# biotite-dev/springcraft

Measured on AMD Instinct MI355X. Metric: ANM modes/sec (Hessian build + full eigensolve), N=2000 C-alpha, higher is better.
Workload: dtype f64; 1 GPU; C3: N=2000 C-alpha ANM, HinsenForceField (no cutoff), full 6000x6000 eigensolve, all modes + vectors; parallelism=independent structures sharded over GPUs, no data-path collective

## Files before the change

### include/springcraft_hip_debug.h

```cpp
#ifndef SPRINGCRAFT_HIP_DEBUG_H
#define SPRINGCRAFT_HIP_DEBUG_H

#include "springcraft_hip.h"

#ifdef __cplusplus
extern "C" {
#endif

int sc_dbg_gemm_bench(sc_ctx* ctx, int m, int n, int k, int mode, int tile, int split_k, int iters, int beta_one,
                      double* ms_out, double* max_err_out);

int sc_dbg_gemm_host(sc_ctx* ctx, const double* a, const double* b, double* c, int m, int n, int k, int mode, int tile,
                     int split_k, double alpha, double beta, int lower_grid);

typedef struct sc_dbg_gemm_record {
  long long a, b, c;
  long long a_kidx, b_kidx, c_jidx;
  long long sa_i, sa_k, sb_k, sb_j, ldc, split_stride;
  double alpha, beta;
  int m, n, k;
  int lower_only, row_off, col_off;
  int a_tri;
  int reserved;
} sc_dbg_gemm_record;

int sc_dbg_gemm_records_host(sc_ctx* ctx, double* arena, long long arena_len, const int* idx, long long idx_len,
                             const sc_dbg_gemm_record* recs, int count, int max_m, int max_n, int split_k, int gather,
                             int tri, int layout, int lower_grid, int tile);

int sc_dbg_gemm3_host(sc_ctx* ctx, const double* a, const double* b, double* c, int count, int m, int n, int k, int layout,
                      int lower, double beta);

int sc_dbg_symm3_host(sc_ctx* ctx, const double* a, const double* v, double* x, int count, int m, int split);
int sc_dbg_symm3_stamps(unsigned long long* out4);
int sc_dbg_symm3_bench(sc_ctx* ctx, int count, int m, int split, int iters, double* ms_out);

int sc_dbg_gemm3_bench(sc_ctx* ctx, int count, int m, int n, int k, int layout, int lower, int kernel, int order, int iters,
                       double* ms_out);

int sc_dbg_gemm_stamps(unsigned long long* out4, int reset);

int sc_dbg_gemm_trace(unsigned long long* out, int max_records, int* count, int reset);

int sc_dbg_reduce_host(sc_ctx* ctx, const double* a, int n, int batch, int which, double* d_out, double* e_out,
                       double* scale_out, double* band_out, double* q_out, int* two_stage_out);

int sc_dbg_stedc_host(sc_ctx* ctx, const double* d, const double* e, int n, int batch, double* w_out, double* z_out);
int sc_dbg_stedc_leaf_max(int n);

int sc_dbg_partial_tridiag_host(sc_ctx* ctx, const double* d, const double* e, const double* f, const int* own, int n,
                                int batch, int window, int il, int m, double vl, double vu, int vectors, double* w_out,
                                double* z_out, int* win_out, long long* count_out);

int sc_dbg_bt2_stamps(unsigned long long* out);

int sc_dbg_bt2_clock(unsigned long long* out2);

int sc_dbg_bt2_trace(unsigned long long* out);

int sc_dbg_bulge_stamps(unsigned long long* out6);
int sc_dbg_pair_stamps(unsigned long long* out48);
int sc_dbg_chase_stamps(unsigned long long* out16);

int sc_dbg_set_chase(sc_ctx* ctx, int mode, int give_up_after);

int sc_dbg_set_panel_coop(sc_ctx* ctx, int min_rows);
int sc_dbg_set_panel_coop_fail(sc_ctx* ctx, int panel);

int sc_dbg_set_resident(sc_ctx* ctx, int mode, int hook, int workgroups);
int sc_dbg_resident_stamps(unsigned long long* out8);

#ifdef __cplusplus
}
#endif
#endif
```

### springcraft_amd/csrc/gemm_debug.hip

```cpp
#include <algorithm>
#include <cmath>
#include <cstdlib>
#include <vector>

#include "gemm_f64.h"
#include "springcraft_hip_debug.h"

namespace {
struct FirstError {
  sc_ctx* ctx;
  int rc = SC_OK;
  void operator()(hipError_t e) { if (e != hipSuccess && rc == SC_OK) rc = sc_set_error(ctx, SC_ERR_HIP, "%s", hipGetErrorString(e)); }
};

struct Shape {
  sc_ctx* ctx;
  int count;
  size_t ea, eb, ec;
  FirstError fail{ctx};
  char* base = nullptr;
  double *a = nullptr, *b = nullptr, *c = nullptr;
  GemmDesc* d = nullptr;
  ~Shape() { (void)hipFree(base); }
  int alloc() {
// ... 167 lines not shown
  if (R.ldc < R.m) return "ldc < m";
  if (R.k > 0) {
    if ((wide)R.a + (wide)(R.m - 1) * R.sa_i + (wide)ka * R.sa_k >= (wide)arena_len) return "A reaches outside the arena";
    if ((wide)R.b + (wide)kb * R.sb_k + (wide)(R.n - 1) * R.sb_j >= (wide)arena_len) return "B reaches outside the arena";
  }
  if ((wide)R.c + (wide)(L.split_k - 1) * R.split_stride + (wide)jc * R.ldc + (R.m - 1) >= (wide)arena_len)
    return "C reaches outside the arena";
  return nullptr;
}
}

extern "C" int sc_dbg_gemm_records_host(sc_ctx* ctx, double* arena, long long arena_len, const int* idx, long long idx_len,
                                        const sc_dbg_gemm_record* recs, int count, int max_m, int max_n, int split_k,
                                        int gather, int tri, int layout, int lower_grid, int tile) {
  if (!ctx) return SC_ERR_INVALID_ARG;
  if (!arena || arena_len <= 0 || arena_len > (1ll << 34) || idx_len < 0 || idx_len > (1ll << 34) || (idx_len > 0 && !idx) ||
      !recs || count < 0 || count > (1 << 24) || max_m <= 0 || max_n <= 0 || split_k < 1 || split_k > 65535)
    return sc_set_error(ctx, SC_ERR_INVALID_ARG, "GEMM records: bad launch argument");
  if (tile < 10 || tile > 13) return sc_set_error(ctx, SC_ERR_INVALID_ARG, "tile id %d (10 .. 13)", tile);
  if (layout < 0 || layout > 2 || (gather && (tri || layout != kGemmAmBk)) || (tri && layout == kGemmAmBn))
    return sc_set_error(ctx, SC_ERR_INVALID_ARG, "GEMM records: no kernel for layout %d, gather %d, tri %d", layout, gather, tri);
  if (lower_grid && (layout != kGemmAmBn || tri || gather || split_k > 1 || max_m != max_n))
    return sc_set_error(ctx, SC_ERR_INVALID_ARG, "GEMM records: lower_grid is for square launches of layout kGemmAmBn without split-K");
  const GemmLaunch L{.count = count, .max_m = max_m, .max_n = max_n, .layout = layout, .split_k = split_k, .gather = gather != 0,
                     .tri = tri != 0, .lower_grid = lower_grid != 0, .dbg = {.force_tile = tile - 10}};
  for (int r = 0; r < count; ++r) {
    const char* what = gemm_record_problem(recs[r], arena_len, idx, idx_len, L);
    if (what) return sc_set_error(ctx, SC_ERR_INVALID_ARG, "GEMM record %d: %s", r, what);
  }
  SC_HIP(ctx, hipSetDevice(ctx->device));
  auto up = [](size_t b) { return (b + 255) / 256 * 256; };
  const size_t b_arena = up((size_t)(arena_len + 2 * kRecGuard) * 8), b_desc = up((size_t)std::max(count, 1) * sizeof(GemmDesc));
  const size_t b_idx = up((size_t)std::max<long long>(idx_len, 1) * 4);
  char* base = nullptr;
  SC_HIP(ctx, hipMalloc((void**)&base, b_arena + b_desc + b_idx));
  double *d_front = (double*)base, *d_arena = d_front + kRecGuard, *d_back = d_arena + arena_len;
  GemmDesc* d_desc = (GemmDesc*)(base + b_arena);
  int* d_idx = (int*)(base + b_arena + b_desc);
  FirstError fail{ctx};
  std::vector<unsigned long long> guard((size_t)kRecGuard, kRecGuardBits), got((size_t)kRecGuard);
  fail(hipMemcpy(d_front, guard.data(), (size_t)kRecGuard * 8, hipMemcpyHostToDevice));
  fail(hipMemcpy(d_back, guard.data(), (size_t)kRecGuard * 8, hipMemcpyHostToDevice));
  fail(hipMemcpy(d_arena, arena, (size_t)arena_len * 8, hipMemcpyHostToDevice));
  if (idx_len > 0) fail(hipMemcpy(d_idx, idx, (size_t)idx_len * 4, hipMemcpyHostToDevice));
  std::vector<GemmDesc> h_desc((size_t)count);
  for (int r = 0; r < count; ++r) {
    const sc_dbg_gemm_record& R = recs[r];
    GemmDesc& D = h_desc[(size_t)r];
    D = GemmDesc{};
    D.a = d_arena + R.a; D.b = d_arena + R.b; D.c = d_arena + R.c;
    D.m = R.m; D.n = R.n; D.k = R.k;
    D.sa_i = R.sa_i; D.sa_k = R.sa_k; D.sb_k = R.sb_k; D.sb_j = R.sb_j; D.ldc = R.ldc;
    D.alpha = R.alpha; D.beta = R.beta;
    D.a_kidx = R.a_kidx >= 0 ? d_idx + R.a_kidx : nullptr;
    D.b_kidx = R.b_kidx >= 0 ? d_idx + R.b_kidx : nullptr;
    D.c_jidx = R.c_jidx >= 0 ? d_idx + R.c_jidx : nullptr;
    D.lower_only = R.lower_only; D.row_off = R.row_off; D.col_off = R.col_off;
    D.split_stride = R.split_stride; D.a_tri = R.a_tri;
  }
  if (count > 0) fail(hipMemcpy(d_desc, h_desc.data(), (size_t)count * sizeof(GemmDesc), hipMemcpyHostToDevice));
  if (fail.rc == SC_OK) {
    fail.rc = launch_gemm_f64(ctx, d_desc, L);
    fail(hipStreamSynchronize(ctx->stream));
  }
  if (fail.rc == SC_OK) fail(hipMemcpy(arena, d_arena, (size_t)arena_len * 8, hipMemcpyDeviceToHost));
  for (double* g : {d_front, d_back}) {
    if (fail.rc != SC_OK) break;
    fail(hipMemcpy(got.data(), g, (size_t)kRecGuard * 8, hipMemcpyDeviceToHost));
    if (fail.rc == SC_OK && got != guard) fail.rc = sc_set_error(ctx, SC_ERR_HIP, "GEMM records: the launch wrote outside the arena");
  }
  (void)hipFree(base);
  return fail.rc;
}

extern "C" int sc_dbg_gemm3_host(sc_ctx* ctx, const double* a, const double* b, double* c, int count, int m, int n, int k,
                                 int layout, int lower, double beta) {
  if (!ctx || !a || !b || !c || count < 1 || m < 1 || n < 1 || k < 1) return SC_ERR_INVALID_ARG;
  Shape S{ctx, count, (size_t)m * k, (size_t)k * n, (size_t)m * n};
  SC_TRY(S.alloc());
  S.fail(hipMemcpy(S.a, a, S.ea * count * 8, hipMemcpyHostToDevice));
  S.fail(hipMemcpy(S.b, b, S.eb * count * 8, hipMemcpyHostToDevice));
  S.fail(hipMemcpy(S.c, c, S.ec * count * 8, hipMemcpyHostToDevice));
  S.upload(gemm3_record(m, n, k, layout, lower, beta, m, n, m));
  if (S.fail.rc == SC_OK) {
    const int took = launch_gemm3_uniform(ctx, S.d, {.count = count, .m = m, .n = n, .k = k, .layout = layout, .lower = lower, .alpha = 1.0,
                                                     .beta = beta, .aligned16 = true, .dbg = {.any_size = true}});
    if (took != SC_OK) S.fail.rc = sc_set_error(ctx, SC_ERR_INVALID_ARG, "k_gemm3 does not take m %d n %d k %d layout %d", m, n, k, layout);
    S.fail(hipStreamSynchronize(ctx->stream));
  }
  if (S.fail.rc == SC_OK) S.fail(hipMemcpy(c, S.c, S.ec * count * 8, hipMemcpyDeviceToHost));
  return S.fail.rc;
}

extern "C" int sc_dbg_gemm3_bench(sc_ctx* ctx, int count, int m, int n, int k, int layout, int lower, int kernel, int order,
                                  int iters, double* ms_out) {
  if (!ctx || count < 1 || iters < 1) return SC_ERR_INVALID_ARG;
  static const int ld_a = [] { const char* e = getenv("SC_DBG_LDA"); return e ? atoi(e) : 0; }();
  static const int ld_c = [] { const char* e = getenv("SC_DBG_LDC"); return e ? atoi(e) : 0; }();
  static const int ld_b = [] { const char* e = getenv("SC_DBG_LDB"); return e ? atoi(e) : 0; }();
  const int lda = std::max(m, ld_a), ldc = std::max(m, ld_c), ldbn = std::max(n, ld_b);
  Shape S{ctx, count, (size_t)lda * k, layout == kGemmAmBn ? (size_t)ldbn * k : (size_t)k * n, (size_t)ldc * n};
  SC_TRY(S.alloc());
  S.fill_random();
  S.fail(hipMemset(S.c, 0, S.ec * count * 8));
  S.upload(gemm3_record(m, n, k, layout, lower, 1.0, lda, ldbn, ldc));
  if (S.fail.rc != SC_OK) return S.fail.rc;
  return S.time(2, iters, ms_out, [&]() -> int {
    if (kernel != 3)
      return launch_gemm_f64(ctx, S.d, {.count = count, .max_m = m, .max_n = n, .layout = layout, .lower_grid = lower != 0 && layout == kGemmAmBn});
    const int took = launch_gemm3_uniform(ctx, S.d, {.count = count, .m = m, .n = n, .k = k, .layout = layout, .lower = lower, .alpha = 1.0,
                                                     .beta = 1.0, .aligned16 = true, .dbg = {.any_size = true, .order = order}});
    return took == SC_OK ? SC_OK : SC_ERR_INVALID_ARG;
  });
}

extern "C" int sc_dbg_symm3_host(sc_ctx* ctx, const double* a, const double* v, double* x, int count, int m, int split) {
  if (!ctx || !a || !v || !x || count < 1 || m < 1 || split < 1) return SC_ERR_INVALID_ARG;
  const size_t ev = (size_t)m * 64;
  Shape S{ctx, count, (size_t)m * m, ev, ev * split};
  SC_TRY(S.alloc());
  S.fail(hipMemcpy(S.a, a, S.ea * count * 8, hipMemcpyHostToDevice));
  S.fail(hipMemcpy(S.b, v, ev * count * 8, hipMemcpyHostToDevice));
  S.fail(hipMemset(S.c, 0xff, S.ec * count * 8));
  S.upload(symm3_record(m));
  if (S.fail.rc == SC_OK) {
    const int took = launch_symm3(ctx, S.d, count, m, split, true, true);
    if (took != SC_OK) S.fail.rc = sc_set_error(ctx, SC_ERR_INVALID_ARG, "k_symm3 does not take m %d split %d", m, split);
    S.fail(hipStreamSynchronize(ctx->stream));
  }
  if (S.fail.rc == SC_OK) {
    std::vector<double> hx(S.ec * count);
    S.fail(hipMemcpy(hx.data(), S.c, hx.size() * 8, hipMemcpyDeviceToHost));
    for (int z = 0; z < count; ++z)
      for (size_t e = 0; e < ev; ++e) {
        double s = 0.0;
        for (int q = 0; q < split; ++q) s += hx[(size_t)z * S.ec + (size_t)q * ev + e];
        x[(size_t)z * ev + e] = s;
      }
  }
  return S.fail.rc;
}

extern "C" int sc_dbg_symm3_bench(sc_ctx* ctx, int count, int m, int split, int iters, double* ms_out) {
  if (!ctx || count < 1 || iters < 1 || m < 256) return SC_ERR_INVALID_ARG;
  Shape S{ctx, count, (size_t)m * m, (size_t)m * 64, (size_t)m * 64 * split};
  SC_TRY(S.alloc());
  S.fill_random();
  S.upload(symm3_record(m));
  if (S.fail.rc != SC_OK) return S.fail.rc;
  return S.time(2, iters, ms_out, [&] {
    return launch_symm3(ctx, S.d, count, m, split, true, true) == SC_OK ? SC_OK : SC_ERR_INVALID_ARG;
  });
}
```

### springcraft_amd/csrc/gemm_f64.h

```cpp
#pragma once

#include <cstdint>

#include "common.h"
#include "gemm_policy.h"

struct GemmDesc {
  const double* a;
  const double* b;
  double* c;
  int m, n, k;
  long long sa_i, sa_k;
  long long sb_k, sb_j;
  long long ldc;
  double alpha, beta;
  const int* a_kidx;
  const int* b_kidx;
  const int* c_jidx;
  int lower_only;
  int row_off, col_off;
  long long split_stride;
  int a_tri;
};

using sc_host::GemmLaunch, sc_host::Gemm3Launch, sc_host::GemmOverrides;
int launch_gemm_f64(sc_ctx* ctx, const GemmDesc* d_desc, const GemmLaunch& L);
int gemm_f64_tile(const sc_ctx* ctx, int count, int max_m, int max_n, int layout);
inline sc_host::GemmDevice gemm_device(const sc_ctx* ctx) { return {ctx->num_cus, ctx->gemm3_attr, ctx->gemm3_side_by_side}; }

int launch_gemm3_uniform(sc_ctx* ctx, const GemmDesc* d_desc, const Gemm3Launch& L);
bool gemm3_would_take(sc_ctx* ctx, const Gemm3Launch& L);

int launch_symm3(sc_ctx* ctx, const GemmDesc* d_desc, int count, int m, int split, bool aligned16, bool any_size);
bool symm3_would_take(sc_ctx* ctx, int count, int m, int split, bool aligned16);
```

### springcraft_amd/csrc/sy2sb.hip

```cpp
#include <algorithm>
#include <vector>

#include "twostage_internal.h"

namespace {

constexpr int kEarly = (kIb + 2) / 2;

__global__ __launch_bounds__(256) void k_panel_qr(double* __restrict__ a_all, long long stride_a,
                                                  double* __restrict__ tri_all, TriLayout TL,
                                                  double* __restrict__ sb_all, SbLayout SL, int j0, int j, int nr,
                                                  int c_end) {
  constexpr int LD = kQrRows + 1;
  extern __shared__ __attribute__((aligned(16))) double sm[];
  const int c_lo = j > 0 ? j - 1 : 0;
  const int ncl = c_end - c_lo;
  double* P = sm;
  double* wv = sm + ncl * LD;
  double* vv = wv + kB;
  double* red = vv + kQrRows;
  __shared__ double s_scale, s_beta, s_tau;

  const int n = TL.n;
  const int r0 = j0 + kB, m = n - r0;
// ... 1056 lines not shown
      GemmDesc P{};
      P.a = sb + SL.xv + (size_t)2 * kB * n + r0; P.sa_i = n; P.sa_k = 1;
      P.b = sb + SL.xv + r0; P.sb_k = 1; P.sb_j = n;
      P.c = sb + SL.small; P.ldc = kB;
      P.m = kB; P.n = 3 * kB; P.k = m; P.alpha = 1.0; P.beta = 0.0;
      P.split_stride = (long long)kB * 3 * kB;
      g[2] = P;
      GemmDesc W{};
      W.a = sb + SL.xv + r0; W.sa_i = 1; W.sa_k = n;
      W.b = sb + SL.cmat; W.sb_k = 1; W.sb_j = 3 * kB;
      W.c = sb + SL.vw + (size_t)vw_w * n + r0; W.ldc = n;
      W.m = m; W.n = kB; W.k = 3 * kB; W.alpha = 1.0; W.beta = 0.0;
      g[3] = W;
      W.c = sb + SL.wv + (size_t)wv_w * n + r0;
      W.alpha = -1.0;
      g[4] = W;
      GemmDesc R{};
      R.a = sb + SL.vw + r0; R.sa_i = 1; R.sa_k = n;
      R.b = sb + SL.wv + r0; R.sb_k = n; R.sb_j = 1;
      R.c = a22; R.ldc = n;
      R.m = m; R.n = m; R.k = rl == 2 ? 4 * kB : 2 * kB; R.alpha = 1.0; R.beta = 1.0;
      R.lower_only = sc_host::symm3_for(E, n) ? 2 : 1;
      g[5] = R;
      GemmDesc D = R;
      D.n = kB; D.k = 2 * kB;
      g[6] = D;
      GemmDesc Q{};
      Q.a = sb + SL.wv + r0; Q.sa_i = n; Q.sa_k = 1;
      Q.b = sb + SL.xv + (size_t)2 * kB * n + r0; Q.sb_k = 1; Q.sb_j = n;
      Q.c = sb + SL.small2; Q.ldc = 2 * kB;
      Q.m = 2 * kB; Q.n = kB; Q.k = m; Q.alpha = 1.0; Q.beta = 0.0;
      Q.split_stride = (long long)2 * kB * kB;
      g[7] = Q;
      GemmDesc Cr{};
      Cr.a = sb + SL.vw + r0; Cr.sa_i = 1; Cr.sa_k = n;
      Cr.b = sb + SL.p2; Cr.sb_k = 1; Cr.sb_j = 2 * kB;
      Cr.c = sb + SL.xv + r0; Cr.ldc = n;
      Cr.m = m; Cr.n = kB; Cr.k = 2 * kB; Cr.alpha = 1.0; Cr.beta = 1.0;
      g[8] = Cr;
    }
  }
  std::vector<GemmDesc> hs(h.size());
  for (int p = 0; p < npanels; ++p)
    for (int b = 0; b < batch; ++b) {
      const GemmDesc* g = &h[((size_t)p * batch + b) * kDescKinds];
      GemmDesc* o = &hs[(size_t)p * kDescKinds * batch];
      for (int kd = 0; kd < kDescKinds; ++kd) o[(size_t)kd * batch + b] = g[kd];
    }
  return hs;
}

struct PanelRun {
  sc_ctx* ctx;
  hipStream_t st;
  double* d_a; long long stride_a; int n, batch;
  double* d_tri_ws; const TriLayout& TL;
  double* d_sb_ws; const SbLayout& SL;
  const GemmDesc* d_descs;
  const std::vector<int>& role;
  sc_host::CoopPlan coop;
  v4i* coop_recs;
  int* coop_ctl;
  bool use_symm3;
  int symm3_nb_min;
  SbTimers& t;
};

static int run_panel(const PanelRun& R, int p, int lo, int hi, hipStream_t ps, bool timed) {
  using sc_host::PanelQr;
  const sc_host::TwoStageEnv& E = sc_host::two_stage_env();
  sc_ctx* ctx = R.ctx;
  const TriLayout& TL = R.TL;
  const SbLayout& SL = R.SL;
  const int n = R.n, batch = R.batch;
  const long long stride_a = R.stride_a;
  struct StreamScope {
    sc_ctx* c; hipStream_t old;
    StreamScope(sc_ctx* c_, hipStream_t s) : c(c_), old(c_->stream) { c->stream = s; }
    ~StreamScope() { c->stream = old; }
  } scope(ctx, ps);
  const int nb = hi - lo;
  const int rl = R.role[(size_t)p];
  double* a_h = R.d_a + (size_t)lo * stride_a;
  double* tri_h = R.d_tri_ws + (size_t)lo * TL.slab;
  double* sb_h = R.d_sb_ws + (size_t)lo * SL.slab;
  const int j0 = p * kB, r0 = j0 + kB, m = n - r0;
  const int nr = std::min(kB, m - 1);
  const int nchunks = (m + kQrRows - 1) / kQrRows;
  const dim3 qgrid((unsigned)nchunks, (unsigned)nb);
  SbLayout SQ = SL;
  if (rl == 2) { SQ.vw += (long long)2 * kB * n; SQ.wv += (long long)2 * kB * n; }
  if (timed) R.t.qr.start();
  const sc_host::PanelQrForm F = sc_host::panel_qr_form(E, R.coop, R.coop_recs != nullptr, m, nb, ps == R.st);
  switch (F.kind) {
    case PanelQr::Coop: {
      const int coop_g = F.coop_g;
      if (p == ctx->coop_fail_panel) SC_HIP(ctx, hipMemsetAsync(R.coop_ctl + 8 * lo, 1, sizeof(int) * 8 * nb, ps));
      hipLaunchKernelGGL(k_panel_coop, dim3((unsigned)coop_g, (unsigned)nb), dim3(kCoopRows), kCoopLdsBytes, ps, a_h, stride_a,
                         tri_h, TL, sb_h, SQ, j0, coop_g, R.coop_recs + (size_t)lo * coop_recs_per_matrix(coop_g),
                         R.coop_ctl + 8 * lo, (p + 1) * 128);
      hipLaunchKernelGGL(k_panel_serial, dim3((unsigned)nb), dim3(1024), 0, ps, a_h, stride_a, tri_h, TL, sb_h, SQ, j0,
                         (const int*)(R.coop_ctl + 8 * lo), ctx->d_status);
      ++ctx->cnt_coop_launches;
      break;
    }
    case PanelQr::Wg1024: {
      const size_t lds_wg = sizeof(double) * (size_t)(2 * kWgWaves * 8 + 16 + 8 + 8 * kB + kWgWaves * kB * 8);
      const dim3 g1((unsigned)nb), b1((unsigned)kWgThreads);
      ++ctx->cnt_panel_form[std::max(1, std::min(F.ru, 4)) - 1];
      if (F.ru == 1) hipLaunchKernelGGL((k_panel_wg<1, 8>), g1, b1, lds_wg, ps, a_h, stride_a, tri_h, TL, sb_h, SQ, j0);
      else if (F.ru == 2) hipLaunchKernelGGL((k_panel_wg<2, 8>), g1, b1, lds_wg, ps, a_h, stride_a, tri_h, TL, sb_h, SQ, j0);
      else if (F.ru == 3) hipLaunchKernelGGL((k_panel_wg<3, 4>), g1, b1, lds_wg, ps, a_h, stride_a, tri_h, TL, sb_h, SQ, j0);
      else hipLaunchKernelGGL((k_panel_wg<4, 2>), g1, b1, lds_wg, ps, a_h, stride_a, tri_h, TL, sb_h, SQ, j0);
      break;
    }
    case PanelQr::Wg512: {
      constexpr int kW = 512 / 64;
      const size_t lds_wg = sizeof(double) * (size_t)(2 * kW * 8 + 16 + 8 + 8 * kB + kW * kB * 8);
      const dim3 g1((unsigned)nb), b1(512u);
      ++ctx->cnt_panel_form[F.ru == 10 ? 4 : 5];
      if (F.ru == 10) hipLaunchKernelGGL((k_panel_wg<10, 1, 512>), g1, b1, lds_wg, ps, a_h, stride_a, tri_h, TL, sb_h, SQ, j0);
      else hipLaunchKernelGGL((k_panel_wg<12, 1, 512>), g1, b1, lds_wg, ps, a_h, stride_a, tri_h, TL, sb_h, SQ, j0);
      break;
    }
    case PanelQr::Blocked: {
      const size_t lds_qr_blk = sizeof(double) * ((size_t)(kIb + 1) * (kQrRows + 1) + kB + kQrRows + 4 * kB);
      const size_t lds_blk_a = sizeof(double) * ((size_t)kB * (kQrRows + 1) + kQrRows + 8 * kB);
      const size_t lds_blk_b = sizeof(double) * ((size_t)kB * (kQrRows + 1) + kIb * kB + 4 * kB);
      ++ctx->cnt_panel_form[6];
      hipLaunchKernelGGL(k_panel_qr, qgrid, dim3(256), lds_qr_blk, ps, a_h, stride_a, tri_h, TL, sb_h, SQ, j0, 0, nr, kIb);
      for (int c0 = 0; c0 < kB; c0 += kIb) {
        for (int j = c0 + 1; j < c0 + kIb; ++j)
          hipLaunchKernelGGL(k_panel_qr, qgrid, dim3(256), lds_qr_blk, ps, a_h, stride_a, tri_h, TL, sb_h, SQ, j0, j, nr,
                             c0 + kIb);
        const size_t cut = sizeof(double) * (size_t)c0 * (kQrRows + 1);
        hipLaunchKernelGGL(k_pqr_blk_a, qgrid, dim3(256), lds_blk_a - cut, ps, a_h, stride_a, tri_h, TL, sb_h, SQ, j0, c0);
        if (c0 + kIb < kB)
          hipLaunchKernelGGL(k_pqr_blk_b, qgrid, dim3(256), lds_blk_b - cut, ps, a_h, stride_a, tri_h, TL, sb_h, SQ, j0, c0);
      }
      break;
    }
    case PanelQr::Unblocked: {
      const size_t lds_qr = sizeof(double) * ((size_t)kB * (kQrRows + 1) + kB + kQrRows + 4 * kB);
      ++ctx->cnt_panel_form[7];
      for (int j = 0; j <= nr; ++j)
        hipLaunchKernelGGL(k_panel_qr, qgrid, dim3(256), lds_qr, ps, a_h, stride_a, tri_h, TL, sb_h, SQ, j0, j, nr, kB);
      break;
    }
  }
  if (timed) R.t.qr.stop();
  if (rl != 0) ++ctx->cnt_panel_role[rl - 1];
  const GemmDesc* g = R.d_descs + (size_t)p * kDescKinds * batch;
  if (timed) R.t.symm.start();
  if (R.use_symm3 && symm3_would_take(ctx, R.symm3_nb_min, m, SL.symm_split, true) &&
      launch_symm3(ctx, g + lo, nb, m, SL.symm_split, true, true) == SC_OK) {
    if (SL.symm_split > 1)
      hipLaunchKernelGGL(k_sum_xslices, dim3((unsigned)((m + 255) / 256), kB, (unsigned)nb), dim3(256), 0, ps, sb_h, SL, r0);
  } else {
    ++ctx->cnt_symm_tri;
    SC_TRY(launch_gemm_f64(ctx, g + lo, {.count = nb, .max_m = m, .max_n = kB, .layout = kGemmAmBk, .split_k = SL.symm_split, .tri = true}));
    SC_TRY(launch_gemm_f64(ctx, g + batch + lo, {.count = nb, .max_m = m, .max_n = kB, .layout = kGemmAkBk, .split_k = SL.symm_split, .tri = true}));
    if (SL.symm_split > 1)
      hipLaunchKernelGGL(k_sum_xslices, dim3((unsigned)((m + 255) / 256), 2 * kB, (unsigned)nb), dim3(256), 0, ps, sb_h, SL, r0);
  }
  if (rl == 2) {
    SC_TRY(launch_gemm_f64(ctx, g + 7 * batch + lo, {.count = nb, .max_m = 2 * kB, .max_n = kB, .layout = kGemmAkBk, .split_k = kSmallSplit}));
    hipLaunchKernelGGL(k_sum_p2, dim3((unsigned)(2 * kB * kB / 256), (unsigned)nb), dim3(256), 0, ps, sb_h, SL);
    SC_TRY(launch_gemm_f64(ctx, g + 8 * batch + lo, {.count = nb, .max_m = m, .max_n = kB, .layout = kGemmAmBk}));
  }
  if (timed) R.t.symm.stop();
  SC_TRY(launch_gemm_f64(ctx, g + 2 * batch + lo, {.count = nb, .max_m = kB, .max_n = 3 * kB, .layout = kGemmAkBk, .split_k = kSmallSplit}));
  const size_t lds_small = sizeof(double) * 4 * kB * (kB + 1);
  hipLaunchKernelGGL(k_sb_small, dim3((unsigned)nb), dim3(1024), lds_small, ps, tri_h, TL, sb_h, SL, j0);
  if (nb == batch) {
    SC_TRY(launch_gemm_f64(ctx, g + 3 * batch, {.count = 2 * batch, .max_m = m, .max_n = kB, .layout = kGemmAmBk}));
  } else {
    SC_TRY(launch_gemm_f64(ctx, g + 3 * batch + lo, {.count = nb, .max_m = m, .max_n = kB, .layout = kGemmAmBk}));
    SC_TRY(launch_gemm_f64(ctx, g + 4 * batch + lo, {.count = nb, .max_m = m, .max_n = kB, .layout = kGemmAmBk}));
  }
  if (timed) R.t.syr2k.start();
  if (rl == 1)
    SC_TRY(launch_gemm_f64(ctx, g + 6 * batch + lo, {.count = nb, .max_m = m, .max_n = kB, .layout = kGemmAmBn}));
  else
    if (launch_gemm3_uniform(ctx, g + 5 * batch + lo,
                             {.count = nb, .m = m, .n = m, .k = rl == 2 ? 4 * kB : 2 * kB, .layout = kGemmAmBn, .lower = R.use_symm3 ? 2 : 1,
                              .alpha = 1.0, .beta = 1.0, .aligned16 = (n & 1) == 0 && (r0 & 1) == 0}) != SC_OK) {
      ++ctx->cnt_gemm3_declined;
      SC_TRY(launch_gemm_f64(ctx, g + 5 * batch + lo, {.count = nb, .max_m = m, .max_n = m, .layout = kGemmAmBn, .lower_grid = true}));
    }
  if (timed) R.t.syr2k.stop();
  return SC_OK;
}

int sb_stage1(sc_ctx* ctx, double* d_a, long long stride_a, int n, int batch, double* d_tri_ws, const TriLayout& TL,
              double* d_sb_ws, const SbLayout& SL, const GemmDesc* d_descs, const std::vector<int>& role, bool prof,
              SbTimers& timers) {
  const sc_host::TwoStageEnv& E = sc_host::two_stage_env();
  hipStream_t st = ctx->stream;
  const int npanels = (int)role.size();

  for (int b = 0; b < batch; ++b)
    SC_HIP(ctx, hipMemsetAsync(d_tri_ws + (size_t)b * TL.slab + TL.tau, 0, sizeof(double) * n, st));

  const int s1_parts = sc_host::stage1_parts(E, batch, prof);
  ctx->last_stage1_parts = s1_parts;
  ctx->last_symm_slices = SL.symm_split;
  const sc_host::CoopPlan coop = sc_host::coop_plan(E, n, batch, ctx->num_cus, prof, ctx->coop_min_rows, ctx->coop_ok);
  v4i* coop_recs = nullptr;
  int* coop_ctl = nullptr;
  if (coop.ask) {
    if (ctx->coop_attr < 0)
      ctx->coop_attr = hipFuncSetAttribute(reinterpret_cast<const void*>(&k_panel_coop),
                                           hipFuncAttributeMaxDynamicSharedMemorySize, (int)kCoopLdsBytes) == hipSuccess;
    if (ctx->coop_attr == 1 && coop.nb_max >= 1) {
      const size_t rec_bytes = (size_t)batch * coop_recs_per_matrix(coop.gmax) * sizeof(v4i);
      const size_t ctl_bytes = align_up((size_t)batch * 8 * sizeof(int), 256);
      SC_TRY(sc_reserve_dc_aux(ctx, ctl_bytes + rec_bytes));
      coop_ctl = reinterpret_cast<int*>(ctx->dc_aux);
      coop_recs = reinterpret_cast<v4i*>(reinterpret_cast<char*>(ctx->dc_aux) + ctl_bytes);
      SC_HIP(ctx, hipMemsetAsync(ctx->dc_aux, 0, ctl_bytes + rec_bytes, st));
    }
  }
  const bool use_symm3 = sc_host::symm3_for(E, n);
  if (use_symm3)
    for (int b = 0; b < batch; ++b)
      SC_HIP(ctx, hipMemsetAsync(d_sb_ws + (size_t)b * SL.slab + SL.xv + (size_t)kB * n, 0, sizeof(double) * (size_t)kB * n, st));
  const PanelRun R{ctx, st, d_a, stride_a, n, batch, d_tri_ws, TL, d_sb_ws, SL, d_descs, role, coop, coop_recs, coop_ctl,
                   use_symm3, std::max(1, batch / s1_parts), timers};
  if (s1_parts > 1) {
    struct SideBySide {
      sc_ctx* c;
      explicit SideBySide(sc_ctx* c_) : c(c_) { c->gemm3_side_by_side = true; }
      ~SideBySide() { c->gemm3_side_by_side = false; }
    } side_by_side(ctx);
    SC_TRY(sc_aux_stream(ctx));
    SC_TRY(sc_side_streams(ctx, s1_parts - 1));
    SC_HIP(ctx, hipEventRecord(ctx->aux_fork, st));
    for (int q = 1; q < s1_parts; ++q) SC_HIP(ctx, hipStreamWaitEvent(ctx->side_streams[q - 1], ctx->aux_fork, 0));
    int rc_parts = SC_OK;
    for (int p = 0; p < npanels && rc_parts == SC_OK; ++p)
      for (int q = 0; q < s1_parts && rc_parts == SC_OK; ++q) {
        const int lo = (int)((long long)batch * q / s1_parts), hi = (int)((long long)batch * (q + 1) / s1_parts);
        rc_parts = run_panel(R, p, lo, hi, q == 0 ? st : ctx->side_streams[q - 1], q == 0);
      }
    for (int q = 1; q < s1_parts; ++q) {
      SC_HIP(ctx, hipEventRecord(ctx->side_joins[q - 1], ctx->side_streams[q - 1]));
      SC_HIP(ctx, hipStreamWaitEvent(st, ctx->side_joins[q - 1], 0));
    }
    SC_TRY(rc_parts);
  } else {
    for (int p = 0; p < npanels; ++p) SC_TRY(run_panel(R, p, 0, batch, st, true));
  }
  SC_HIP(ctx, hipGetLastError());
  return SC_OK;
}
```

### springcraft_amd/csrc/twostage_policy.h

```cpp
#pragma once
#include <algorithm>
#include <cstddef>
#include <cstdlib>
#include <vector>

#if defined(__HIPCC__)
#define SC_POLICY_HD __host__ __device__
#else
#define SC_POLICY_HD
#endif

namespace sc_host {

constexpr int kBand = 64;
constexpr int kWgRows1024 = 4 * 1024;
constexpr int kWgRows512 = 12 * 512;
constexpr int kCoopRows = 256;
constexpr int kCoopMaxG = 128;
constexpr int kEarlyRing = 8;

static inline size_t policy_align_up(size_t x, size_t a) { return (x + a - 1) / a * a; }

SC_POLICY_HD inline int chase_len(int n, int s) { return (n - 1 - s + kBand - 1) / kBand; }

struct TwoStageEnv {
  int symm3 = 1;
  int symm_split = 0;
  bool panel_pairs = true;
  bool qr_blocked = true;
  int qr_wg = -1;
  int qr_coop = 1;
  int qr_coop_min = 0;
  int stage1_streams = 0;
  int bulge_persistent = 1;
  int bulge_pair = -1;
  long long bulge_pair_max = 6000;
  int bulge_spread = -1;
  bool bulge_no_early = false;
  int bulge_streams = 0;
  int bulge_burst = 32;
  int bt2_wave = -1;
  int bt2_nw = 0;
};

static inline TwoStageEnv read_two_stage_env() {
  TwoStageEnv E;
  auto num = [](const char* name, int unset) { const char* e = getenv(name); return e ? atoi(e) : unset; };
  E.symm3 = num("SPRINGCRAFT_SYMM3", 1);
  E.symm_split = num("SPRINGCRAFT_SYMM_SPLIT", 0);
  E.panel_pairs = num("SPRINGCRAFT_PANEL_PAIRS", 1) != 0;
  E.qr_blocked = getenv("SPRINGCRAFT_QR_UNBLOCKED") == nullptr;
  E.qr_wg = num("SPRINGCRAFT_QR_WG", -1);
  E.qr_coop = num("SPRINGCRAFT_QR_COOP", 1);
  if (const char* e = getenv("SPRINGCRAFT_QR_COOP_MIN")) E.qr_coop_min = std::max(2 * kBand, atoi(e));
  E.stage1_streams = num("SPRINGCRAFT_STAGE1_STREAMS", 0);
  E.bulge_persistent = num("SPRINGCRAFT_BULGE_PERSISTENT", 1);
  E.bulge_pair = num("SPRINGCRAFT_BULGE_PAIR", -1);
  if (const char* e = getenv("SPRINGCRAFT_BULGE_PAIR_MAX")) E.bulge_pair_max = atoll(e);
  E.bulge_spread = num("SPRINGCRAFT_BULGE_SPREAD", -1);
  E.bulge_no_early = getenv("SPRINGCRAFT_BULGE_NO_EARLY") != nullptr;
  E.bulge_streams = num("SPRINGCRAFT_BULGE_STREAMS", 0);
  E.bulge_burst = std::max(1, num("SPRINGCRAFT_BULGE_BURST", 32));
  E.bt2_wave = num("SPRINGCRAFT_BT2_WAVE", -1);
  E.bt2_nw = num("SPRINGCRAFT_BT2_NW", 0);
  return E;
}
inline const TwoStageEnv& two_stage_env() {
  static const TwoStageEnv E = read_two_stage_env();
  return E;
}


static inline int stage1_parts(const TwoStageEnv& E, int batch, bool profiled) {
  const int want = E.stage1_streams > 0 ? E.stage1_streams : ((batch >= 32 && !profiled) ? 2 : 1);
  return std::max(1, std::min(want, std::min(batch, 4)));
}

static inline int panel_count(int n) {
  int npanels = 0;
  while (n - (npanels + 1) * kBand >= 2) ++npanels;
  return npanels;
}
static inline std::vector<int> panel_roles(const TwoStageEnv& E, int n) {
  const int npanels = panel_count(n);
  std::vector<int> role((size_t)npanels, 0);
  if (E.panel_pairs)
    for (int p = 0; p + 1 < npanels;) {
      const int m2 = n - (p + 2) * kBand;
      if (m2 >= 4 * kBand) { role[(size_t)p] = 1; role[(size_t)p + 1] = 2; p += 2; }
      else ++p;
    }
  return role;
}

static inline bool symm3_for(const TwoStageEnv& E, int n) { return E.symm3 != 0 && n >= 512 && (n & 1) == 0; }

static inline int symm_split_for(const TwoStageEnv& E, int n, int batch) {
  if (E.symm_split >= 1) return std::min(E.symm_split, 16);
  if (symm3_for(E, n)) {
    const long long items = (long long)((n + 127) / 128) * (batch >= 32 ? batch / 2 : batch);
    if (items >= 768) return 1;
    return (int)std::min<long long>(16, (1536 + items - 1) / items);
  }
  const long long tiles = (long long)batch * ((n + 63) / 64);
  if (tiles >= 1024 || n < 2048) return 1;
  const long long s0 = std::min<long long>(6, (2048 + tiles - 1) / tiles);
  return s0 >= 6 ? 9 : (s0 == 4 ? 5 : (int)s0);
}

struct CoopPlan {
  bool ask;
  int nb_max;
  int min_few;
  int min_many;
  int budget;
  int gmax;
};
static inline CoopPlan coop_plan(const TwoStageEnv& E, int n, int batch, int num_cus, bool profiled, int coop_min_rows,
                                 int coop_ok) {
  CoopPlan C{};
  C.min_few = coop_min_rows > 0 ? coop_min_rows : (E.qr_coop_min > 0 ? E.qr_coop_min : 300);
  C.min_many = coop_min_rows > 0 ? coop_min_rows : (E.qr_coop_min > 0 ? E.qr_coop_min : kWgRows512 + 1);
  C.budget = num_cus * 3 / 4;
  C.gmax = (std::max(n - kBand, 1) + kCoopRows - 1) / kCoopRows;
  C.ask = (coop_min_rows > 0 || (coop_min_rows < 0 && E.qr_coop != 0)) && coop_ok != 0 &&
          n - kBand >= std::min(C.min_few, C.min_many) && C.gmax <= kCoopMaxG && stage1_parts(E, batch, profiled) == 1;
  C.nb_max = std::min(batch, C.budget / C.gmax);
  return C;
}

enum class PanelQr {
  Coop,
  Wg1024,
  Wg512,
  Blocked,
  Unblocked,
};
struct PanelQrForm {
  PanelQr kind;
  int ru, cu;
  int coop_g;
};
static inline PanelQrForm panel_qr_form(const TwoStageEnv& E, const CoopPlan& C, bool have_recs, int m, int nb,
                                        bool main_stream) {
  PanelQrForm F{PanelQr::Unblocked, 0, 0, (m + kCoopRows - 1) / kCoopRows};
  const bool full = std::min(kBand, m - 1) == kBand;
  const bool use_wg = full && m <= kWgRows1024 && E.qr_wg != 0;
  const bool use_wg512 = full && !use_wg && m <= kWgRows512 && E.qr_wg != 0 && E.qr_wg != 1 && nb >= 4;
  const bool use_coop = have_recs && full && m >= (nb < 4 ? C.min_few : C.min_many) && nb * F.coop_g <= C.budget && main_stream;
  if (use_coop) {
    F.kind = PanelQr::Coop;
  } else if (use_wg) {
    F.kind = PanelQr::Wg1024;
    const int ru = (m + 1023) / 1024;
    F.ru = ru <= 1 ? 1 : std::min(ru, 4);
    F.cu = ru <= 2 ? 8 : (ru == 3 ? 4 : 2);
  } else if (use_wg512) {
    F.kind = PanelQr::Wg512;
    F.ru = (m + 511) / 512 <= 10 ? 10 : 12;
    F.cu = 1;
  } else if (full && E.qr_blocked) {
    F.kind = PanelQr::Blocked;
  }
  return F;
}


enum class ChaseForm {
  Stepwise,
  Sweep,
  Spread,
  Pair,
};
static inline ChaseForm chase_form_for(const TwoStageEnv& E, int n, int batch, int nxcd, int num_cus, bool pair_attr,
                                       int chase_mode, int chase_form, int chase_ok) {
  const int persist = chase_mode >= 0 ? chase_mode : E.bulge_persistent;
  const long long work = (long long)batch * n / 128;
  const bool pair_measured = work <= E.bulge_pair_max && (batch + nxcd - 1) / nxcd <= std::max(1, num_cus / nxcd);
  const bool pair = chase_form >= 0 ? (chase_form == 1 && pair_attr)
                                    : E.bulge_pair != 0 && pair_attr &&
                                          (E.bulge_pair == 2 || (work > 1100 && batch >= 8 && pair_measured));
  const bool spread = !pair && batch < nxcd &&
                      (chase_form == 2 || (chase_form < 0 && E.bulge_spread != 0 && (E.bulge_spread == 1 || n > 4500)));
  const bool want_chase = persist == 2 || (persist == 1 && (pair || spread || (work <= 2800 && (batch >= 8 || n <= 6144))));
  if (!(want_chase && num_cus > 0 && (chase_ok != 0 || persist == 2))) return ChaseForm::Stepwise;
  return pair ? ChaseForm::Pair : (spread ? ChaseForm::Spread : ChaseForm::Sweep);
}

struct ChaseLaunch {
  int nxcd;
  int W;
  int grid;
  size_t prog_bytes;
  size_t next_bytes;
  size_t early_bytes;
};
static inline ChaseLaunch chase_launch(const TwoStageEnv& E, ChaseForm form, int n, int batch, int nxcd_device, int num_cus,
                                       int per_cu) {
  const bool pair = form == ChaseForm::Pair;
  ChaseLaunch L{};
  L.nxcd = form == ChaseForm::Spread ? 1 : nxcd_device;
  const int slots_per_xcd = per_cu * num_cus / L.nxcd;
  const int mpx = (batch + L.nxcd - 1) / L.nxcd;
  const int useful = pair ? std::max(4, chase_len(n, 0) / 3 + 2) : std::max(8, chase_len(n, 0) / 2 + 1);
  L.W = slots_per_xcd > 0 ? std::max(1, std::min(useful, slots_per_xcd / mpx)) : 0;
  L.grid = L.nxcd * std::min(slots_per_xcd, mpx * L.W);
  L.prog_bytes = policy_align_up((size_t)batch * n * sizeof(int), 256);
  L.next_bytes = policy_align_up((size_t)batch * sizeof(int), 256);
// ... 34 lines not shown
```

Baseline: 180,400 modes/s.

## Add specialized skinny MFMA kernels for panel-update GEMMs in band reduction

Adds dedicated f64 MFMA kernels for the tall-skinny A^T·B products (split-K slices with optional zeroing of known-zero blocks) and In·C products (C staged in LDS, writing both positive and negated outputs in one pass). The sy2sb panel update uses them instead of the general GEMM when enabled, which is the default. It also skips multiplying a block that is known to be zero when symm3 ran. The goal is to cut launch count and wasted work on small-N panel GEMMs in stage-1 reduction. Correctness now depends on the zero-block assumption and on the fixed 64-wide tile shapes.

```diff
diff --git a/include/springcraft_hip_debug.h b/include/springcraft_hip_debug.h
--- a/include/springcraft_hip_debug.h
+++ b/include/springcraft_hip_debug.h
@@ -34,6 +34,11 @@
 int sc_dbg_symm3_host(sc_ctx* ctx, const double* a, const double* v, double* x, int count, int m, int split);
 int sc_dbg_symm3_stamps(unsigned long long* out4);
 int sc_dbg_symm3_bench(sc_ctx* ctx, int count, int m, int split, int iters, double* ms_out);
+
+int sc_dbg_skinny_tn_f64(sc_ctx* ctx, const double* a, const double* b, double* s, int count, int m, int ld, int row_off,
+                         int p, int nblk, unsigned zero_mask, int slices_buf, int slices_used, int* used_out);
+int sc_dbg_skinny_nn_f64(sc_ctx* ctx, const double* in, const double* cmat, double* out, double* out_neg, int count, int m,
+                         int ld, int row_off, int kblocks, int nb, const int* blk);
 
 int sc_dbg_gemm3_bench(sc_ctx* ctx, int count, int m, int n, int k, int layout, int lower, int kernel, int order, int iters,
                        double* ms_out);
diff --git a/springcraft_amd/csrc/gemm_debug.hip b/springcraft_amd/csrc/gemm_debug.hip
--- a/springcraft_amd/csrc/gemm_debug.hip
+++ b/springcraft_amd/csrc/gemm_debug.hip
@@ -343,3 +343,78 @@
     return launch_symm3(ctx, S.d, count, m, split, true, true) == SC_OK ? SC_OK : SC_ERR_INVALID_ARG;
   });
 }
+
+extern "C" int sc_dbg_skinny_tn_f64(sc_ctx* ctx, const double* a, const double* b, double* s, int count, int m, int ld,
+                                    int row_off, int p, int nblk, unsigned zero_mask, int slices_buf, int slices_used,
+                                    int* used_out) {
+  if (!ctx || !a || !b || !s || count < 1 || m < 1 || row_off < 0 || (long long)row_off + m > ld || (p != 64 && p != 128) || nblk < 1 ||
+      nblk > 3 || slices_buf < 1 || slices_buf > 64 || slices_used < 0 || slices_used > slices_buf)
+    return SC_ERR_INVALID_ARG;
+  const size_t q = (size_t)64 * nblk;
+  Shape S{ctx, count, (size_t)ld * p, (size_t)ld * q, (size_t)p * q * slices_buf};
+  SC_TRY(S.alloc());
+  S.fail(hipMemcpy(S.a, a, S.ea * count * 8, hipMemcpyHostToDevice));
+  S.fail(hipMemcpy(S.b, b, S.eb * count * 8, hipMemcpyHostToDevice));
+  S.fail(hipMemcpy(S.c, s, S.ec * count * 8, hipMemcpyHostToDevice));
+  std::vector<GemmDesc> h((size_t)count);
+  for (int z = 0; z < count; ++z) {
+    GemmDesc D{};
+    D.a = S.a + S.ea * z + row_off; D.sa_i = ld; D.sa_k = 1;
+    D.b = S.b + S.eb * z + row_off; D.sb_k = 1; D.sb_j = ld;
+    D.c = S.c + S.ec * z; D.ldc = p; D.split_stride = (long long)(p * q);
+    D.m = p; D.n = (int)q; D.k = m; D.alpha = 1.0;
+    h[(size_t)z] = D;
+  }
+  S.fail(hipMemcpy(S.d, h.data(), sizeof(GemmDesc) * (size_t)count, hipMemcpyHostToDevice));
+  const int used = slices_used > 0 ? slices_used : skinny_tn_slices(ctx, count, m, slices_buf);
+  if (used_out) *used_out = used;
+  if (S.fail.rc == SC_OK) {
+    S.fail.rc = launch_skinny_tn(ctx, S.d, count, m, p, nblk, zero_mask, slices_buf, used);
+    S.fail(hipStreamSynchronize(ctx->stream));
+  }
+  if (S.fail.rc == SC_OK) S.fail(hipMemcpy(s, S.c, S.ec * count * 8, hipMemcpyDeviceToHost));
+  return S.fail.rc;
+}
+
+extern "C" int sc_dbg_skinny_nn_f64(sc_ctx* ctx, const double* in, const double* cmat, double* out, double* out_neg, int count,
+                                    int m, int ld, int row_off, int kblocks, int nb, const int* blk) {
+  if (!ctx || !in || !cmat || !out || !blk || count < 1 || m < 1 || row_off < 0 || (long long)row_off + m > ld || kblocks < 2 ||
+      kblocks > 3 || (nb != 2 && nb != 3) || nb > kblocks)
+    return SC_ERR_INVALID_ARG;
+  for (int t = 0; t < nb; ++t)
+    if (blk[t] < 0 || blk[t] >= kblocks) return SC_ERR_INVALID_ARG;
+  const size_t k = (size_t)64 * kblocks, eo = (size_t)ld * 64;
+  Shape S{ctx, count, (size_t)ld * k, k * 64, 2 * eo};
+  SC_TRY(S.alloc());
+  S.fail(hipMemcpy(S.a, in, S.ea * count * 8, hipMemcpyHostToDevice));
+  S.fail(hipMemcpy(S.b, cmat, S.eb * count * 8, hipMemcpyHostToDevice));
+  for (int z = 0; z < count; ++z) {
+    S.fail(hipMemcpy(S.c + S.ec * z, out + eo * z, eo * 8, hipMemcpyHostToDevice));
+    if (out_neg) S.fail(hipMemcpy(S.c + S.ec * z + eo, out_neg + eo * z, eo * 8, hipMemcpyHostToDevice));
+  }
+  char* neg_base = nullptr;
+  S.fail(hipMalloc((void**)&neg_base, sizeof(GemmDesc) * (size_t)count));
+  std::vector<GemmDesc> h((size_t)count), hn((size_t)count);
+  for (int z = 0; z < count; ++z) {
+    GemmDesc D{};
+    D.a = S.a + S.ea * z + row_off; D.sa_i = 1; D.sa_k = ld;
+    D.b = S.b + S.eb * z; D.sb_k = 1; D.sb_j = (long long)k;
+    D.c = S.c + S.ec * z + row_off; D.ldc = ld;
+    D.m = m; D.n = 64; D.k = (int)k; D.alpha = 1.0; D.beta = out_neg ? 0.0 : 1.0;
+    h[(size_t)z] = D;
+    D.c += eo; D.alpha = -1.0;
+    hn[(size_t)z] = D;
+  }
+  S.fail(hipMemcpy(S.d, h.data(), sizeof(GemmDesc) * (size_t)count, hipMemcpyHostToDevice));
+  if (neg_base) S.fail(hipMemcpy(neg_base, hn.data(), sizeof(GemmDesc) * (size_t)count, hipMemcpyHostToDevice));
+  if (S.fail.rc == SC_OK) {
+    S.fail.rc = launch_skinny_nn(ctx, S.d, out_neg ? reinterpret_cast<const GemmDesc*>(neg_base) : nullptr, count, m, nb, blk);
+    S.fail(hipStreamSynchronize(ctx->stream));
+  }
+  for (int z = 0; z < count && S.fail.rc == SC_OK; ++z) {
+    S.fail(hipMemcpy(out + eo * z, S.c + S.ec * z, eo * 8, hipMemcpyDeviceToHost));
+    if (out_neg) S.fail(hipMemcpy(out_neg + eo * z, S.c + S.ec * z + eo, eo * 8, hipMemcpyDeviceToHost));
+  }
+  (void)hipFree(neg_base);
+  return S.fail.rc;
+}
diff --git a/springcraft_amd/csrc/gemm_f64.h b/springcraft_amd/csrc/gemm_f64.h
--- a/springcraft_amd/csrc/gemm_f64.h
+++ b/springcraft_amd/csrc/gemm_f64.h
@@ -33,3 +33,8 @@
 
 int launch_symm3(sc_ctx* ctx, const GemmDesc* d_desc, int count, int m, int split, bool aligned16, bool any_size);
 bool symm3_would_take(sc_ctx* ctx, int count, int m, int split, bool aligned16);
+
+int skinny_tn_slices(const sc_ctx* ctx, int count, int m, int cap);
+int launch_skinny_tn(sc_ctx* ctx, const GemmDesc* d_desc, int count, int m, int p, int nblk, unsigned zero_mask,
+                     int slices_buf, int slices_used);
+int launch_skinny_nn(sc_ctx* ctx, const GemmDesc* d_desc, const GemmDesc* d_neg, int count, int m, int nb, const int* blk);
diff --git a/springcraft_amd/csrc/skinny.hip b/springcraft_amd/csrc/skinny.hip
--- /dev/null
+++ b/springcraft_amd/csrc/skinny.hip
@@ -0,0 +1,225 @@
+#include <algorithm>
+
+#include "gemm_f64.h"
+
+namespace {
+
+typedef double d4 __attribute__((ext_vector_type(4)));
+
+struct SkinnyTn {
+  const GemmDesc* d;
+  int rps;
+  int bsel[3];
+  int nblk;
+  unsigned zero_mask;
+};
+
+template <int PT, int QB>
+__global__ __launch_bounds__(256) void k_skinny_tn(SkinnyTn A) {
+  const GemmDesc& D = A.d[blockIdx.y];
+  const int tid = threadIdx.x, w = tid >> 6, l = tid & 63, lr = l & 15, lq = l >> 4;
+  const int m = D.k;
+  const int lo = (int)std::min<long long>((long long)blockIdx.x * A.rps, m), end = std::min(m, lo + A.rps);
+  double* __restrict__ S = D.c + (size_t)blockIdx.x * D.split_stride;
+  const long long ldc = D.ldc;
+
+#pragma unroll
+  for (int blk = 0; blk < 3; ++blk)
+    if (blk < A.nblk && ((A.zero_mask >> blk) & 1u))
+      for (int e = tid; e < 16 * PT * 64; e += 256) S[(size_t)(blk * 64 + e / (16 * PT)) * ldc + e % (16 * PT)] = 0.0;
+
+  const double* ap[PT];
+  const double* bp[QB];
+#pragma unroll
+  for (int a = 0; a < PT; ++a) ap[a] = D.a + (size_t)(a * 16 + lr) * D.sa_i + 4 * lq;
+#pragma unroll
+  for (int q = 0; q < QB; ++q) bp[q] = D.b + (size_t)(A.bsel[q] * 64 + w * 16 + lr) * D.sb_j + 4 * lq;
+
+  d4 acc[QB][PT];
+#pragma unroll
+  for (int q = 0; q < QB; ++q)
+#pragma unroll
+    for (int a = 0; a < PT; ++a) acc[q][a] = d4{0.0, 0.0, 0.0, 0.0};
+
+  auto load = [&](double (&fa)[PT][4], double (&fb)[QB][4], int k0) {
+    if (k0 + 16 <= end) {
+#pragma unroll
+      for (int a = 0; a < PT; ++a)
+#pragma unroll
+        for (int t = 0; t < 4; ++t) fa[a][t] = ap[a][k0 + t];
+#pragma unroll
+      for (int q = 0; q < QB; ++q)
+#pragma unroll
+        for (int t = 0; t < 4; ++t) fb[q][t] = bp[q][k0 + t];
+    } else {
+      const int left = end - k0 - 4 * lq;
+#pragma unroll
+      for (int a = 0; a < PT; ++a)
+#pragma unroll
+        for (int t = 0; t < 4; ++t) fa[a][t] = t < left ? ap[a][k0 + t] : 0.0;
+#pragma unroll
+      for (int q = 0; q < QB; ++q)
+#pragma unroll
+        for (int t = 0; t < 4; ++t) fb[q][t] = t < left ? bp[q][k0 + t] : 0.0;
+    }
+  };
+  auto mma = [&](const double (&fa)[PT][4], const double (&fb)[QB][4]) {
+#pragma unroll
+    for (int t = 0; t < 4; ++t)
+#pragma unroll
+      for (int q = 0; q < QB; ++q)
+#pragma unroll
+        for (int a = 0; a < PT; ++a) acc[q][a] = __builtin_amdgcn_mfma_f64_16x16x4f64(fa[a][t], fb[q][t], acc[q][a], 0, 0, 0);
+  };
+
+  if (lo < end) {
+    double fa0[PT][4], fb0[QB][4], fa1[PT][4], fb1[QB][4];
+    load(fa0, fb0, lo);
+    for (int k0 = lo; k0 < end; k0 += 32) {
+      if (k0 + 16 < end) load(fa1, fb1, k0 + 16);
+      mma(fa0, fb0);
+      if (k0 + 16 >= end) break;
+      if (k0 + 32 < end) load(fa0, fb0, k0 + 32);
+      mma(fa1, fb1);
+    }
+  }
+
+#pragma unroll
+  for (int q = 0; q < QB; ++q) {
+    double* col = S + (size_t)(A.bsel[q] * 64 + w * 16 + lr) * ldc + lq;
+#pragma unroll
+    for (int a = 0; a < PT; ++a)
+#pragma unroll
+      for (int r = 0; r < 4; ++r) col[a * 16 + 4 * r] = acc[q][a][r];
+  }
+}
+
+struct SkinnyNn {
+  const GemmDesc* d;
+  const GemmDesc* d2;
+  int blk[3];
+};
+
+constexpr int skinny_nn_ldk(int nb) { return nb * 64 + 2; }
+constexpr int skinny_nn_lds(int nb) { return 64 * skinny_nn_ldk(nb) * (int)sizeof(double); }
+
+template <int NB, bool ACCUMULATE>
+__global__ __launch_bounds__(256) void k_skinny_nn(SkinnyNn A) {
+  extern __shared__ __attribute__((aligned(16))) double sC[];
+  constexpr int LDK = skinny_nn_ldk(NB);
+  const GemmDesc& D = A.d[blockIdx.y];
+  const int tid = threadIdx.x, w = tid >> 6, l = tid & 63, lr = l & 15, lq = l >> 4;
+  const int m = D.m;
+#pragma unroll
+  for (int b = 0; b < NB; ++b) {
+    const double* src = D.b + (size_t)A.blk[b] * 64;
+    for (int e = tid; e < 64 * 64; e += 256) sC[(e >> 6) * LDK + b * 64 + (e & 63)] = src[(size_t)(e >> 6) * D.sb_j + (e & 63)];
+  }
+  __syncthreads();
+  const int row0 = (int)blockIdx.x * 128 + w * 32;
+  if (row0 >= m) return;
+  const bool ok[2] = {row0 + lr < m, row0 + 16 + lr < m};
+  const double* ip[2];
+#pragma unroll
+  for (int rt = 0; rt < 2; ++rt) ip[rt] = D.a + (size_t)lq * D.sa_k + row0 + rt * 16 + lr;
+  const long long lda = D.sa_k;
+
+  d4 acc[2][4];
+#pragma unroll
+  for (int rt = 0; rt < 2; ++rt)
+#pragma unroll
+    for (int ct = 0; ct < 4; ++ct) acc[rt][ct] = d4{0.0, 0.0, 0.0, 0.0};
+
+  double x[2][2][16];
+  auto load = [&](double (&f)[2][16], int b) {
+    const size_t off = (size_t)A.blk[b] * 64 * lda;
+#pragma unroll
+    for (int s = 0; s < 16; ++s)
+#pragma unroll
+      for (int rt = 0; rt < 2; ++rt) f[rt][s] = ok[rt] ? ip[rt][off + (size_t)(4 * s) * lda] : 0.0;
+  };
+  load(x[0], 0);
+#pragma unroll
+  for (int b = 0; b < NB; ++b) {
+    if (b + 1 < NB) load(x[(b + 1) & 1], b + 1);
+#pragma unroll
+    for (int s = 0; s < 16; ++s) {
+      double cf[4];
+#pragma unroll
+      for (int ct = 0; ct < 4; ++ct) cf[ct] = sC[(ct * 16 + lr) * LDK + b * 64 + 4 * s + lq];
+#pragma unroll
+      for (int rt = 0; rt < 2; ++rt)
+#pragma unroll
+        for (int ct = 0; ct < 4; ++ct) acc[rt][ct] = __builtin_amdgcn_mfma_f64_16x16x4f64(cf[ct], x[b & 1][rt][s], acc[rt][ct], 0, 0, 0);
+    }
+  }
+
+  double* __restrict__ c1 = D.c;
+  const long long ldc = D.ldc;
+#pragma unroll
+  for (int rt = 0; rt < 2; ++rt) {
+    if (!ok[rt]) continue;
+    const int row = row0 + rt * 16 + lr;
+#pragma unroll
+    for (int ct = 0; ct < 4; ++ct)
+#pragma unroll
+      for (int r = 0; r < 4; ++r) {
+        const size_t col = (size_t)(ct * 16 + 4 * r + lq);
+        const double v = acc[rt][ct][r];
+        if constexpr (ACCUMULATE) {
+          c1[col * ldc + row] += v;
+        } else {
+          c1[col * ldc + row] = v;
+          A.d2[blockIdx.y].c[col * A.d2[blockIdx.y].ldc + row] = -v;
+        }
+      }
+  }
+}
+
+}
+
+int skinny_tn_slices(const sc_ctx* ctx, int count, int m, int cap) {
+  const int cus = ctx->num_cus > 0 ? ctx->num_cus : 256;
+  const int want = (2 * cus + std::max(count, 1) - 1) / std::max(count, 1);
+  return std::max(1, std::min({cap, want, (m + 63) / 64}));
+}
+
+int launch_skinny_tn(sc_ctx* ctx, const GemmDesc* d_desc, int count, int m, int p, int nblk, unsigned zero_mask,
+                     int slices_buf, int slices_used) {
+  if (count <= 0) return SC_OK;
+  if (m < 1 || nblk < 1 || nblk > 3 || slices_buf < 1 || slices_buf > 65535 || slices_used < 1 || slices_used > slices_buf || count > 65535)
+    return sc_set_error(ctx, SC_ERR_INVALID_ARG, "skinny A^T B: m %d, %d blocks, %d of %d slices, %d records", m, nblk, slices_used, slices_buf, count);
+  SkinnyTn A{d_desc, 0, {0, 0, 0}, nblk, zero_mask & ((1u << nblk) - 1u)};
+  A.rps = ((m + slices_used - 1) / slices_used + 15) / 16 * 16;
+  int qb = 0;
+  for (int b = 0; b < nblk; ++b)
+    if (!((A.zero_mask >> b) & 1u)) A.bsel[qb++] = b;
+  const dim3 grid((unsigned)slices_buf, (unsigned)count), block(256);
+  if (p == 64 && qb == 3) hipLaunchKernelGGL((k_skinny_tn<4, 3>), grid, block, 0, ctx->stream, A);
+  else if (p == 64 && qb == 2) hipLaunchKernelGGL((k_skinny_tn<4, 2>), grid, block, 0, ctx->stream, A);
+  else if (p == 64 && qb == 1) hipLaunchKernelGGL((k_skinny_tn<4, 1>), grid, block, 0, ctx->stream, A);
+  else if (p == 128 && qb == 1) hipLaunchKernelGGL((k_skinny_tn<8, 1>), grid, block, 0, ctx->stream, A);
+  else return sc_set_error(ctx, SC_ERR_INVALID_ARG, "skinny A^T B: no kernel for p %d with %d multiplied blocks", p, qb);
+  SC_HIP(ctx, hipGetLastError());
+  return SC_OK;
+}
+
+int launch_skinny_nn(sc_ctx* ctx, const GemmDesc* d_desc, const GemmDesc* d_neg, int count, int m, int nb, const int* blk) {
+  if (count <= 0) return SC_OK;
+  if (m < 1 || (nb != 2 && nb != 3) || count > 65535)
+    return sc_set_error(ctx, SC_ERR_INVALID_ARG, "skinny In C: m %d, %d blocks, %d records", m, nb, count);
+  SkinnyNn A{d_desc, d_neg, {0, 0, 0}};
+  for (int b = 0; b < nb; ++b) A.blk[b] = blk[b];
+  const dim3 grid((unsigned)((m + 127) / 128), (unsigned)count), block(256);
+  const void* fn = nullptr;
+  if (nb == 2) fn = d_neg ? reinterpret_cast<const void*>(&k_skinny_nn<2, false>) : reinterpret_cast<const void*>(&k_skinny_nn<2, true>);
+  else fn = d_neg ? reinterpret_cast<const void*>(&k_skinny_nn<3, false>) : reinterpret_cast<const void*>(&k_skinny_nn<3, true>);
+  const int lds = nb == 2 ? skinny_nn_lds(2) : skinny_nn_lds(3);
+  if (!sc_raise_dyn_lds(fn, lds)) return sc_set_error(ctx, SC_ERR_HIP, "skinny In C: %d bytes of LDS refused", lds);
+  if (nb == 2 && d_neg) hipLaunchKernelGGL((k_skinny_nn<2, false>), grid, block, lds, ctx->stream, A);
+  else if (nb == 2) hipLaunchKernelGGL((k_skinny_nn<2, true>), grid, block, lds, ctx->stream, A);
+  else if (d_neg) hipLaunchKernelGGL((k_skinny_nn<3, false>), grid, block, lds, ctx->stream, A);
+  else hipLaunchKernelGGL((k_skinny_nn<3, true>), grid, block, lds, ctx->stream, A);
+  SC_HIP(ctx, hipGetLastError());
+  return SC_OK;
+}
diff --git a/springcraft_amd/csrc/sy2sb.hip b/springcraft_amd/csrc/sy2sb.hip
--- a/springcraft_amd/csrc/sy2sb.hip
+++ b/springcraft_amd/csrc/sy2sb.hip
@@ -1232,8 +1232,10 @@
   if (rl != 0) ++ctx->cnt_panel_role[rl - 1];
   const GemmDesc* g = R.d_descs + (size_t)p * kDescKinds * batch;
   if (timed) R.t.symm.start();
+  bool x2_zero = false;
   if (R.use_symm3 && symm3_would_take(ctx, R.symm3_nb_min, m, SL.symm_split, true) &&
       launch_symm3(ctx, g + lo, nb, m, SL.symm_split, true, true) == SC_OK) {
+    x2_zero = true;
     if (SL.symm_split > 1)
       hipLaunchKernelGGL(k_sum_xslices, dim3((unsigned)((m + 255) / 256), kB, (unsigned)nb), dim3(256), 0, ps, sb_h, SL, r0);
   } else {
@@ -1243,16 +1245,34 @@
     if (SL.symm_split > 1)
       hipLaunchKernelGGL(k_sum_xslices, dim3((unsigned)((m + 255) / 256), 2 * kB, (unsigned)nb), dim3(256), 0, ps, sb_h, SL, r0);
   }
+  const bool skinny = E.skinny;
+  const int tn_slices = skinny ? skinny_tn_slices(ctx, R.symm3_nb_min, m, kSmallSplit) : 0;
   if (rl == 2) {
-    SC_TRY(launch_gemm_f64(ctx, g + 7 * batch + lo, {.count = nb, .max_m = 2 * kB, .max_n = kB, .layout = kGemmAkBk, .split_k = kSmallSplit}));
+    if (skinny) {
+      SC_TRY(launch_skinny_tn(ctx, g + 7 * batch + lo, nb, m, 2 * kB, 1, 0u, kSmallSplit, tn_slices));
+    } else {
+      SC_TRY(launch_gemm_f64(ctx, g + 7 * batch + lo, {.count = nb, .max_m = 2 * kB, .max_n = kB, .layout = kGemmAkBk, .split_k = kSmallSplit}));
+    }
     hipLaunchKernelGGL(k_sum_p2, dim3((unsigned)(2 * kB * kB / 256), (unsigned)nb), dim3(256), 0, ps, sb_h, SL);
-    SC_TRY(launch_gemm_f64(ctx, g + 8 * batch + lo, {.count = nb, .max_m = m, .max_n = kB, .layout = kGemmAmBk}));
+    if (skinny) {
+      const int both[2] = {0, 1};
+      SC_TRY(launch_skinny_nn(ctx, g + 8 * batch + lo, nullptr, nb, m, 2, both));
+    } else {
+      SC_TRY(launch_gemm_f64(ctx, g + 8 * batch + lo, {.count = nb, .max_m = m, .max_n = kB, .layout = kGemmAmBk}));
+    }
   }
   if (timed) R.t.symm.stop();
-  SC_TRY(launch_gemm_f64(ctx, g + 2 * batch + lo, {.count = nb, .max_m = kB, .max_n = 3 * kB, .layout = kGemmAkBk, .split_k = kSmallSplit}));
+  if (skinny) {
+    SC_TRY(launch_skinny_tn(ctx, g + 2 * batch + lo, nb, m, kB, 3, x2_zero ? 2u : 0u, kSmallSplit, tn_slices));
+  } else {
+    SC_TRY(launch_gemm_f64(ctx, g + 2 * batch + lo, {.count = nb, .max_m = kB, .max_n = 3 * kB, .layout = kGemmAkBk, .split_k = kSmallSplit}));
+  }
   const size_t lds_small = sizeof(double) * 4 * kB * (kB + 1);
   hipLaunchKernelGGL(k_sb_small, dim3((unsigned)nb), dim3(1024), lds_small, ps, tri_h, TL, sb_h, SL, j0);
-  if (nb == batch) {
+  if (skinny) {
+    const int x1_v[2] = {0, 2}, all[3] = {0, 1, 2};
+    SC_TRY(launch_skinny_nn(ctx, g + 3 * batch + lo, g + 4 * batch + lo, nb, m, x2_zero ? 2 : 3, x2_zero ? x1_v : all));
+  } else if (nb == batch) {
     SC_TRY(launch_gemm_f64(ctx, g + 3 * batch, {.count = 2 * batch, .max_m = m, .max_n = kB, .layout = kGemmAmBk}));
   } else {
     SC_TRY(launch_gemm_f64(ctx, g + 3 * batch + lo, {.count = nb, .max_m = m, .max_n = kB, .layout = kGemmAmBk}));
diff --git a/springcraft_amd/csrc/twostage_policy.h b/springcraft_amd/csrc/twostage_policy.h
--- a/springcraft_amd/csrc/twostage_policy.h
+++ b/springcraft_amd/csrc/twostage_policy.h
@@ -32,6 +32,7 @@
   int qr_coop = 1;
   int qr_coop_min = 0;
   int stage1_streams = 0;
+  bool skinny = true;
   int bulge_persistent = 1;
   int bulge_pair = -1;
   long long bulge_pair_max = 6000;
@@ -54,6 +55,7 @@
   E.qr_coop = num("SPRINGCRAFT_QR_COOP", 1);
   if (const char* e = getenv("SPRINGCRAFT_QR_COOP_MIN")) E.qr_coop_min = std::max(2 * kBand, atoi(e));
   E.stage1_streams = num("SPRINGCRAFT_STAGE1_STREAMS", 0);
+  E.skinny = num("SPRINGCRAFT_SKINNY", 1) != 0;
   E.bulge_persistent = num("SPRINGCRAFT_BULGE_PERSISTENT", 1);
   E.bulge_pair = num("SPRINGCRAFT_BULGE_PAIR", -1);
   if (const char* e = getenv("SPRINGCRAFT_BULGE_PAIR_MAX")) E.bulge_pair_max = atoll(e);
```

After: 180,600 modes/s (median of 2 runs). No clear change (+0.1%).
